# OPM/opm-autodiff

Measured on AMD Instinct MI355X. Metric: Newton iterations/sec, 1M-cell 3-phase black-oil (assembly + ILU0/BiCGStab solve + update), higher is better.
Workload: dtype f64

## Files before the change

### opm-autodiff_amd/csrc/capi.cpp

```cpp
#include <cstdlib>
#include <chrono>
#include <unordered_map>
#include <algorithm>
#include <cstring>
#include <new>

#include "internal.hpp"

using namespace opmhip;

namespace {
thread_local std::string g_err = "";

double now() {
    return std::chrono::duration<double>(std::chrono::steady_clock::now().time_since_epoch()).count();
}

int alloc_system(opmhip_ctx* c) {
    const Pattern& P = c->pat;
    const size_t n = (size_t)P.Nloc * BS;
    int rc;
    constexpr size_t SLACK = 2 * BB;
    if ((rc = dev_alloc(c, &c->d_A, (size_t)P.nnzb * BB + SLACK))) return rc;
    if ((rc = dev_alloc(c, &c->d_L, (size_t)P.nl * BB + SLACK))) return rc;
    if ((rc = dev_alloc(c, &c->d_U, (size_t)P.nu * BB + SLACK))) return rc;
    OPMHIP_HIP(c, hipMemsetAsync(c->d_A + (size_t)P.nnzb * BB, 0, SLACK * sizeof(double), c->stream));
    const size_t l0 = P.fillLevel > 0 ? 0 : (size_t)P.nl * BB, u0 = P.fillLevel > 0 ? 0 : (size_t)P.nu * BB;
    OPMHIP_HIP(c, hipMemsetAsync(c->d_L + l0, 0, ((size_t)P.nl * BB + SLACK - l0) * sizeof(double), c->stream));
    OPMHIP_HIP(c, hipMemsetAsync(c->d_U + u0, 0, ((size_t)P.nu * BB + SLACK - u0) * sizeof(double), c->stream));
    if ((rc = dev_alloc(c, &c->d_invD, (size_t)P.Nb * BB))) return rc;
    c->half_product = half_product_wanted(c);
    if (c->half_product) {
        if ((rc = dev_alloc(c, &c->d_R, (size_t)P.nr * BB + SLACK))) return rc;
        OPMHIP_HIP(c, hipMemsetAsync(c->d_R, 0, ((size_t)P.nr * BB + SLACK) * sizeof(double), c->stream));
        if ((rc = dev_alloc(c, &c->d_usum, n))) return rc;
        OPMHIP_HIP(c, hipMemsetAsync(c->d_usum, 0, n * sizeof(double), c->stream));
    }
    double** vecs[] = {&c->d_b, &c->d_x, &c->d_r, &c->d_rw, &c->d_p, &c->d_v, &c->d_s, &c->d_t, &c->d_pw, &c->d_vu, &c->d_stageV};
    for (double** v : vecs) {
        if ((rc = dev_alloc(c, v, n))) return rc;
        OPMHIP_HIP(c, hipMemsetAsync(*v, 0, n * sizeof(double), c->stream));
    }
    if ((rc = dev_alloc(c, &c->d_stageA, (size_t)P.nnzb * BB))) return rc;
    if ((rc = dev_alloc(c, &c->d_scal, (size_t)SC_COUNT))) return rc;
    OPMHIP_HIP(c, hipMemsetAsync(c->d_scal, 0, SC_COUNT * sizeof(double), c->stream));
    const int vb = (int)((n + 2047) / 2048);
    c->npart = std::max(std::max(P.tiles.ntiles(), P.tiles.nsched), vb) + 1;
    if ((rc = dev_alloc(c, &c->d_part, (size_t)3 * c->npart))) return rc;
    OPMHIP_HIP(c, hipMemsetAsync(c->d_part, 0, (size_t)3 * c->npart * sizeof(double), c->stream));
    if ((rc = dev_alloc(c, &c->d_part2, (size_t)1024))) return rc;
    OPMHIP_HIP(c, hipMemsetAsync(c->d_part2, 0, 1024 * sizeof(double), c->stream));
    if (!c->h_pinned) OPMHIP_HIP(c, hipHostMalloc((void**)&c->h_pinned, SC_COUNT * sizeof(double)));
    if (!c->h_ring) {
    OPMHIP_HIP(c, hipHostMalloc((void**)&c->h_ring, opmhip_ctx::RB_SLOTS * opmhip_ctx::RB_DOUBLES * sizeof(double), hipHostMallocMapped));
    OPMHIP_HIP(c, hipHostGetDevicePointer((void**)&c->d_ring, c->h_ring, 0));
    std::memset(c->h_ring, 0, opmhip_ctx::RB_SLOTS * opmhip_ctx::RB_DOUBLES * sizeof(double));
    }
    c->d_done = c->d_scal + SC_ZERO;
    OPMHIP_HIP(c, hipStreamSynchronize(c->stream));
    return OPMHIP_SUCCESS;
}

static bool no_standard_wells(const opmhip_ctx* c, const opmhip_wells* w) {
    return !w || (w->num_wells <= 0 && !(w->distributed != 0 && c->comm.nranks > 1));
}

static int upload_wells_local(opmhip_ctx* c, const opmhip_wells* w) {
    WellsDev& W = c->wells;
    if (w->num_ms_wells > 0) {
        if (!w->ms_apply) return fail(c, OPMHIP_INVALID_ARGUMENT, "wells: num_ms_wells = %d but ms_apply == NULL", w->num_ms_wells);
        if (c->comm.nranks > 1) return fail(c, OPMHIP_INVALID_ARGUMENT, "wells: multisegment wells through the host callback are not supported in decomposed runs");
        if (W.ms.num > 0)
            return fail(c, OPMHIP_INVALID_ARGUMENT, "wells: num_ms_wells = %d with a callback while a device-resident list of %d multisegment wells is set "
                        "(opmhip_set_ms_wells): the operator would be applied twice", w->num_ms_wells, W.ms.num);
        const size_t bytes = (size_t)c->pat.Nb * BS * sizeof(double);
        if (!W.h_x) OPMHIP_HIP(c, hipHostMalloc((void**)&W.h_x, bytes));
        if (!W.h_y) OPMHIP_HIP(c, hipHostMalloc((void**)&W.h_y, bytes));
        W.num_ms = w->num_ms_wells;
// ... 204 lines not shown
    cfg->tolerance = 1e-2;
    cfg->ilu_relaxation = 0.9;
    cfg->relax_mode = OPMHIP_RELAX_POST_SCALE;
    cfg->reorder = OPMHIP_REORDER_AUTO;
    cfg->cpr_amg_ilu_levels = -1;
    cfg->zero_diag_fix = 1;
    cfg->cpr_reuse_setup = 3;
}

int opmhip_create(const opmhip_config* cfg, opmhip_ctx** out) {
    if (!out) { g_err = "opmhip_create: out == NULL"; return OPMHIP_INVALID_ARGUMENT; }
    *out = nullptr;
    if (!cfg || cfg->abi_version != OPMHIP_ABI_VERSION) { g_err = "opmhip_create: config missing or ABI version mismatch"; return OPMHIP_INVALID_ARGUMENT; }
    if (cfg->maxit < 1 || !(cfg->tolerance > 0.0)) { g_err = "opmhip_create: maxit/tolerance out of range"; return OPMHIP_INVALID_ARGUMENT; }
    if (cfg->preconditioner < OPMHIP_PRECOND_ILU0 || cfg->preconditioner > OPMHIP_PRECOND_CPR_TRUEIMPES) { g_err = "opmhip_create: unknown preconditioner"; return OPMHIP_INVALID_ARGUMENT; }
    if (cfg->chain_length < 0) { g_err = "opmhip_create: chain_length < 0"; return OPMHIP_INVALID_ARGUMENT; }
    if (cfg->cpr_reuse_setup < 0 || cfg->cpr_reuse_setup > 3) { g_err = "opmhip_create: cpr_reuse_setup must be 0 .. 3"; return OPMHIP_INVALID_ARGUMENT; }
    if (cfg->cpr_async_setup < 0 || cfg->cpr_async_setup > 1) { g_err = "opmhip_create: cpr_async_setup must be 0 or 1"; return OPMHIP_INVALID_ARGUMENT; }
    if (cfg->fused_reductions < 0 || cfg->fused_reductions > 1) { g_err = "opmhip_create: fused_reductions must be 0 or 1"; return OPMHIP_INVALID_ARGUMENT; }
    if (cfg->fused_reductions && cfg->tolerance < 1e-6) { g_err = "opmhip_create: fused_reductions needs tolerance >= 1e-6 (the recurred residual norm cannot resolve less than sqrt(eps) |r_0|)"; return OPMHIP_INVALID_ARGUMENT; }
    if (cfg->pin_host_arrays < 0 || cfg->pin_host_arrays > 1) { g_err = "opmhip_create: pin_host_arrays must be 0 or 1"; return OPMHIP_INVALID_ARGUMENT; }
    int ndev = 0;
    hipError_t e = hipGetDeviceCount(&ndev);
    if (e != hipSuccess || ndev <= 0) {
        g_err = std::string("opmhip_create: no HIP device visible (") + hipGetErrorString(e) + "); libopmhip has no CPU fallback";
        return OPMHIP_NO_DEVICE;
    }
    if (cfg->device_id < 0 || cfg->device_id >= ndev) { g_err = "opmhip_create: device_id out of range"; return OPMHIP_INVALID_ARGUMENT; }
    opmhip_ctx* c = new (std::nothrow) opmhip_ctx();
    if (!c) { g_err = "opmhip_create: out of memory"; return OPMHIP_UNKNOWN_ERROR; }
    c->cfg = *cfg;
    c->device = cfg->device_id;
    if ((e = hipSetDevice(c->device)) != hipSuccess || (e = hipStreamCreateWithFlags(&c->stream, hipStreamNonBlocking)) != hipSuccess ||
        (e = hipEventCreate(&c->ev0)) != hipSuccess || (e = hipEventCreate(&c->ev1)) != hipSuccess) {
        g_err = std::string("opmhip_create: ") + hipGetErrorString(e);
        delete c;
        return OPMHIP_DEVICE_ERROR;
    }
    *out = c;
    return OPMHIP_SUCCESS;
}

void opmhip_destroy(opmhip_ctx* c) {
    if (!c) return;
    (void)hipSetDevice(c->device);
    if (c->stream) (void)hipStreamSynchronize(c->stream);
    cpr_shutdown(c);
    comm_release(c);
    for (const auto& r : c->pinned)
        if (r.bytes) (void)hipHostUnregister(const_cast<void*>(r.p));
    for (void* p : c->allocs) (void)hipFree(p);
    if (c->h_pinned) (void)hipHostFree(c->h_pinned);
    if (c->wells.h_x) (void)hipHostFree(c->wells.h_x);
    if (c->wells.h_y) (void)hipHostFree(c->wells.h_y);
    if (c->wells.ms.h_flag) (void)hipHostFree(c->wells.ms.h_flag);
    if (c->h_ring) (void)hipHostFree(c->h_ring);
    if (c->ev0) (void)hipEventDestroy(c->ev0);
    if (c->ev1) (void)hipEventDestroy(c->ev1);
    for (hipEvent_t e : c->prof.ev) (void)hipEventDestroy(e);
    if (c->stream) (void)hipStreamDestroy(c->stream);
    delete c;
}

const char* opmhip_last_error(const opmhip_ctx* c) { return c ? c->err.c_str() : g_err.c_str(); }

int opmhip_synchronize(opmhip_ctx* c) {
    if (!c) return OPMHIP_INVALID_ARGUMENT;
    OPMHIP_HIP(c, hipSetDevice(c->device));
    OPMHIP_HIP(c, hipStreamSynchronize(c->stream));
    return OPMHIP_SUCCESS;
}

int opmhip_set_pattern(opmhip_ctx* c, int Nb, int nnzb, const int* rows, const int* cols) {
    return opmhip_set_pattern_dd(c, Nb, 0, nnzb, rows, cols);
}

int opmhip_set_pattern_dd(opmhip_ctx* c, int Nb, int Nghost, int nnzb, const int* rows, const int* cols) {
    if (!c) return OPMHIP_INVALID_ARGUMENT;
    return guarded(c, [&]() -> int {
        if (c->pattern_set) return fail(c, OPMHIP_NOT_READY, "set_pattern: the pattern of a context is immutable (linalg/ISTLSolverEbos.hpp:216-219)");
        OPMHIP_HIP(c, hipSetDevice(c->device));
        int rc = build_pattern(c, Nb, Nghost, nnzb, rows, cols);
        if (rc) return rc;
        for (int i = 0; i < Nb; ++i)
            if (rows[i + 1] - rows[i] > TILE_CAP_BLOCKS)
                return fail(c, OPMHIP_ANALYSIS_FAILED, "row %d has %d blocks; the ILU0 tile kernel holds at most %d", i, rows[i + 1] - rows[i], TILE_CAP_BLOCKS);
        if ((rc = alloc_system(c))) return rc;
        c->pattern_set = true;
        return OPMHIP_SUCCESS;
    });
}

int opmhip_upload_system(opmhip_ctx* c, const double* vals, const double* b) {
    if (!c) return OPMHIP_INVALID_ARGUMENT;
    return guarded(c, [&]() -> int {
        if (!c->pattern_set) return fail(c, OPMHIP_NOT_READY, "upload_system before set_pattern");
        OPMHIP_HIP(c, hipSetDevice(c->device));
        int rc = upload_system(c, vals, b);
        if (rc) return rc;
        OPMHIP_HIP(c, hipStreamSynchronize(c->stream));
        return OPMHIP_SUCCESS;
    });
// ... 522 lines not shown
    }
    info[3] = P.rest.on ? P.rest.nsched : 0;
    return OPMHIP_SUCCESS;
}

int opmhip_profile_enable(opmhip_ctx* c, int on) {
    if (!c) return OPMHIP_INVALID_ARGUMENT;
    return guarded(c, [&]() -> int {
        OPMHIP_HIP(c, hipSetDevice(c->device));
        OPMHIP_HIP(c, hipStreamSynchronize(c->stream));
        Profiler& P = c->prof;
        P.enabled = on != 0;
        P.every = on > 1 ? on : 1;
        P.solve_no = 0;
        P.suspended = false;
        P.pending = -1;
        P.used = 0;
        P.ev_used = 0;
        for (int k = 0; k < PROF_COUNT; ++k) { P.total_ms[k] = 0.0; P.count[k] = 0; }
        return OPMHIP_SUCCESS;
    });
}

int opmhip_profile_get(opmhip_ctx* c, int cls, long long* launches, double* total_ms) {
    if (!c) return OPMHIP_INVALID_ARGUMENT;
    return guarded(c, [&]() -> int {
        if (cls < 0 || cls >= PROF_COUNT || !launches || !total_ms) return fail(c, OPMHIP_INVALID_ARGUMENT, "profile_get: bad arguments");
        OPMHIP_HIP(c, hipSetDevice(c->device));
        OPMHIP_HIP(c, hipStreamSynchronize(c->stream));
        Profiler& P = c->prof;
        prof_flush(c);
        OPMHIP_HIP(c, hipStreamSynchronize(c->stream));
        if (c->comm.hstream) OPMHIP_HIP(c, hipStreamSynchronize(c->comm.hstream));
        for (size_t i = 0; i < P.used; ++i) {
            float ms = 0.f;
            if (P.cls[i] >= 0 && P.e1[i] >= 0 && hipEventElapsedTime(&ms, P.ev[P.e0[i]], P.ev[P.e1[i]]) == hipSuccess) {
                P.total_ms[P.cls[i]] += ms;
                P.count[P.cls[i]] += 1;
            }
        }
        P.used = 0;
        P.ev_used = 0;
        *launches = P.count[cls];
        *total_ms = P.total_ms[cls];
        return OPMHIP_SUCCESS;
    });
}

int opmhip_cpr_levels(opmhip_ctx* c, int* n, int* nnz, int cap) {
    if (!c || !n || !nnz || cap < 1) return OPMHIP_INVALID_ARGUMENT;
    return cpr_level_sizes(c, n, nnz, cap);
}

int opmhip_time_kernel(opmhip_ctx* c, int which, int reps, double* ms_per_launch) {
    if (!c) return OPMHIP_INVALID_ARGUMENT;
    return guarded(c, [&]() -> int {
        if (!ms_per_launch || reps < 1 || which < 0 || which > 9) return fail(c, OPMHIP_INVALID_ARGUMENT, "time_kernel: bad arguments");
        if (which >= 7 && !c->half_product) return fail(c, OPMHIP_NOT_READY, "time_kernel: the half-product form is not in force on this context");
        if (!c->system_loaded) return fail(c, OPMHIP_NOT_READY, "time_kernel before a matrix was uploaded");
        if (which != 2 && which != 4 && !c->factored) return fail(c, OPMHIP_NOT_READY, "time_kernel: factor first");
        OPMHIP_HIP(c, hipSetDevice(c->device));
        auto once = [&]() {
            switch (which) {
                case 0: (void)launch_spmv(c, c->d_pw, c->d_v, 0, nullptr); break;
                case 1: launch_ilu_apply(c, c->d_p, c->d_pw); break;
                case 2: launch_ilu_factor(c); break;
                case 3: launch_vector_kernels_once(c); break;
                case 4: launch_stream_read(c); break;
                case 5: (void)launch_spmv(c, c->d_pw, c->d_v, 1, c->d_rw); break;
                case 6: (void)launch_spmv(c, c->d_pw, c->d_v, 2, c->d_r); break;
                case 7: (void)launch_spmv(c, c->d_pw, c->d_v, 0, nullptr, 1.0, false, c->d_usum); break;
// ... 20 lines not shown
```

### opm-autodiff_amd/csrc/internal.hpp

```cpp
#pragma once
#include <hip/hip_runtime.h>

#include <cstdarg>
#include <cstdio>
#include <cstdlib>
#include <cstring>
#include <memory>
#include <climits>
#include <string>
#include <type_traits>
#include <vector>

#include "../../include/opmhip.h"
#include "cpr_setup.hpp"

namespace opmhip {

constexpr int BS = 3;
constexpr int BB = 9;

#ifndef OPMHIP_TILE_ROWS
#define OPMHIP_TILE_ROWS 32
#endif
constexpr int TILE_ROWS = OPMHIP_TILE_ROWS;
// ... 239 lines not shown
    double* d_apg = nullptr;
    std::shared_ptr<CprDev> glob;
};
struct CprDev {
    bool structured = false, coarse_direct = true;
    bool level0 = false;
    std::shared_ptr<CprAsyncJob> job;
    bool recreate = false;
    std::vector<CprLevelDev> lv;
    double *d_w = nullptr, *d_lu = nullptr;
    double* d_pcol = nullptr;
    bool w_given = false;
    double *d_r = nullptr, *d_y = nullptr, *d_z = nullptr;
    double omega = 2.0 / 3.0, damp = 1.6, beta = 0.25;
    CprGatherDev gather;
    int apply_rc = 0;
    bool pvals_fresh = false;
};
struct FactorRider {
    int mode = 0;
    double* w = nullptr;
    double* ap = nullptr;
    double* pcol = nullptr;
    int W = 0;
    int ghostFrom = INT_MAX;
};

enum ProfClass { PROF_SPMV = 0, PROF_ILU_APPLY, PROF_ILU_FACTOR, PROF_VECTOR, PROF_ASSEMBLE, PROF_IQ_UPDATE, PROF_CONVERGENCE, PROF_CPR_AMG,
                 PROF_SPMV_BOUNDARY,
                 PROF_HALO,
                 PROF_ALLREDUCE,
                 PROF_CPR_GATHER,
                 PROF_COUNT };
struct Profiler {
    bool enabled = false;
    int every = 1;
    long solve_no = 0;
    bool suspended = false;
    std::vector<hipEvent_t> ev;
    size_t ev_used = 0;
    std::vector<int> cls, e0, e1;
    size_t used = 0;
    int pending = -1;
    bool lazy = false;
    int handoff = -1;
    static constexpr size_t CAP = 1 << 15;
    double total_ms[PROF_COUNT] = {0};
    long count[PROF_COUNT] = {0};
};

enum Scal {
    SC_RHO = 0, SC_RHOP, SC_ALPHA, SC_OMEGA, SC_BETA, SC_TMP1, SC_TMP2, SC_NORM, SC_NORM0,
    SC_DONE,
    SC_ZERO,
    SC_RR,
    SC_RHOH,
    SC_DONEH,
    SC_COUNT = 16
};

}

struct opmhip_ctx {
    opmhip_config cfg;
    int device = 0;
    hipStream_t stream = nullptr;
    hipEvent_t ev0 = nullptr, ev1 = nullptr;
    std::string err;
    bool pattern_set = false, system_loaded = false, factored = false, have_result = false;
    int ilu_fillin = 0;
    opmhip::Pattern pat;
    double *d_A = nullptr, *d_L = nullptr, *d_U = nullptr, *d_invD = nullptr;
    double *d_R = nullptr, *d_usum = nullptr;
    bool half_product = false;
    double *d_b = nullptr, *d_x = nullptr, *d_r = nullptr, *d_rw = nullptr, *d_p = nullptr, *d_v = nullptr,
           *d_s = nullptr, *d_t = nullptr, *d_pw = nullptr, *d_vu = nullptr;
    double *d_stageA = nullptr, *d_stageV = nullptr;
    double* d_scal = nullptr;
    double* d_part = nullptr;
    double minv_scale = 1.0;
    double* d_part2 = nullptr;
    int npart = 0;
    int last_solve_iterations = 0;
    int last_dot_count = 0;
    double* h_pinned = nullptr;
    static constexpr int RB_SLOTS = 4, RB_DOUBLES = 4;
    double* h_ring = nullptr;
    double* d_ring = nullptr;
    double rb_seq = 0.0;
    double rb_want[RB_SLOTS] = {0, 0, 0, 0};
    const double* d_done = nullptr;
    opmhip::WellsDev wells;
    opmhip::AsmDev asmb;
    opmhip::CommDev comm;
    opmhip::CprDev cpr;
    opmhip::Profiler prof;
    std::vector<void*> allocs;
    struct HostRange { const void* p; size_t bytes; };
    std::vector<HostRange> pinned;
};

namespace opmhip {

inline const char* tuning_env(const char* name) {
    static const bool on = [] { const char* e = std::getenv("OPMHIP_TUNING"); return e && e[0] == '1'; }();
    const char* v = std::getenv(name);
    if (!v) return nullptr;
    if (!on) {
        std::fprintf(stderr, "opmhip: %s is set but OPMHIP_TUNING=1 is not - ignored\n", name);
        return nullptr;
    }
    std::fprintf(stderr, "opmhip: measurement switch %s=%s is in force\n", name, v);
    return v;
// ... 20 lines not shown
inline bool poison_allocations() {
    static const bool on = [] { const char* e = tuning_env("OPMHIP_POISON_ALLOC"); return e && e[0] == '1'; }();
    return on;
}
template <class T>
int dev_alloc(opmhip_ctx* c, T** p, size_t count) {
    void* q = nullptr;
    size_t bytes = (count ? count : 1) * sizeof(T);
    hipError_t e = hipMalloc(&q, bytes);
    if (e != hipSuccess)
        return fail(c, OPMHIP_DEVICE_ERROR, "hipMalloc(%zu) failed: %s", bytes, hipGetErrorString(e));
    if (poison_allocations() && ((e = hipMemset(q, std::is_floating_point<T>::value ? 0xFF : 0x00, bytes)) != hipSuccess || (e = hipDeviceSynchronize()) != hipSuccess)) {
        (void)hipFree(q);
        return fail(c, OPMHIP_DEVICE_ERROR, "hipMemset(%zu) failed: %s", bytes, hipGetErrorString(e));
    }
    c->allocs.push_back(q);
    *p = static_cast<T*>(q);
    return OPMHIP_SUCCESS;
}
template <class T>
void dev_free(opmhip_ctx* c, T** p) {
    if (!*p) return;
    for (size_t i = 0; i < c->allocs.size(); ++i)
        if (c->allocs[i] == (void*)*p) { c->allocs[i] = c->allocs.back(); c->allocs.pop_back(); break; }
    (void)hipFree((void*)*p);
    *p = nullptr;
}
template <class T>
int dev_upload(opmhip_ctx* c, T** p, const std::vector<T>& h) {
    int rc = dev_alloc(c, p, h.size());
    if (rc) return rc;
    if (!h.empty()) OPMHIP_HIP(c, hipMemcpy(*p, h.data(), h.size() * sizeof(T), hipMemcpyHostToDevice));
    return OPMHIP_SUCCESS;
}

inline int prof_event(opmhip_ctx* c, hipStream_t s = nullptr) {
    Profiler& P = c->prof;
    if (P.ev.size() <= P.ev_used) {
        hipEvent_t e;
        if (hipEventCreate(&e) != hipSuccess) return -1;
        P.ev.push_back(e);
    }
    const int i = (int)P.ev_used++;
    (void)hipEventRecord(P.ev[i], s ? s : c->stream);
    return i;
}
inline int prof_event_slot(opmhip_ctx* c) {
    Profiler& P = c->prof;
    if (P.ev.size() <= P.ev_used) {
        hipEvent_t e;
        if (hipEventCreate(&e) != hipSuccess) return -1;
        P.ev.push_back(e);
    }
    return (int)P.ev_used++;
}
inline void prof_flush(opmhip_ctx* c) {
    Profiler& P = c->prof;
    P.handoff = -1;
    if (P.pending < 0) return;
    const int e = prof_event(c);
    if (e >= 0) P.e1[P.pending] = e; else P.cls[P.pending] = -1;
    P.pending = -1;
}
inline int prof_begin(opmhip_ctx* c, int cls) {
    Profiler& P = c->prof;
    if (!P.enabled || P.suspended || P.used >= Profiler::CAP) { prof_flush(c); return -1; }
// ... 109 lines not shown
```

### opm-autodiff_amd/csrc/solver.hip

```cpp
#include <hip/hip_runtime.h>
#include <hip/hip_ext.h>
#include <atomic>

#include <chrono>
#include <cmath>
#include <cstdlib>

#include "internal.hpp"

namespace opmhip {

#ifndef OPMHIP_STAGE_DEPTH
#define OPMHIP_STAGE_DEPTH 16
#endif
typedef double v2d_t __attribute__((ext_vector_type(2)));
__device__ __forceinline__ double2 ld_stream(const double2* p) {
    const v2d_t t = __builtin_nontemporal_load(reinterpret_cast<const v2d_t*>(p));
    return make_double2(t.x, t.y);
}
__device__ __forceinline__ void st_rowsum(double* p, double v) {
    __builtin_nontemporal_store(v, p);
}
__device__ __forceinline__ void stage_doubles(const double* __restrict__ src, double* __restrict__ dst, int n, int lane) {
    const double2* __restrict__ s2 = reinterpret_cast<const double2*>(src);
// ... 1639 lines not shown
#pragma unroll
    for (int u = 0; u < VPT; ++u) {
        const int e = base + u * VB;
        if (e < n) p[e] = (p[e] - omega * __builtin_nontemporal_load(&v[e])) * beta + r[e];
    }
}
template <bool SR = false>
__global__ __launch_bounds__(VB) void k_bicg_upd1(int n, const double* __restrict__ scal, double* __restrict__ r,
                                                  const double* __restrict__ v, double* __restrict__ part, int npart, double half = -1.0) {
    if (scal[SC_DONE] != 0.0 && !(SR && scal[SC_DONEH] == half)) return;
    const double alpha = scal[SC_ALPHA];
    double s = 0.0;
    const int base = blockIdx.x * VB * VPT + threadIdx.x;
#pragma unroll
    for (int u = 0; u < VPT; ++u) {
        const int e = base + u * VB;
        if (e < n) {
            const double re = r[e] - alpha * __builtin_nontemporal_load(&v[e]);
            r[e] = re;
            s += re * re;
        }
    }
    if (!SR) block_partials(s, 0.0, part, npart, 1);
}
__global__ __launch_bounds__(VB) void k_bicg_xhalf(int n, const double* __restrict__ scal, double* __restrict__ x, const double* __restrict__ pw, double ws) {
    const double alpha = scal[SC_ALPHA];
    const int base = blockIdx.x * VB * VPT + threadIdx.x;
#pragma unroll
    for (int u = 0; u < VPT; ++u) {
        const int e = base + u * VB;
        if (e < n) x[e] += alpha * (ws * pw[e]);
    }
}
template <bool SR = false>
__global__ __launch_bounds__(VB) void k_bicg_upd2(int n, const double* __restrict__ scal, double* __restrict__ x,
                                                  const double* __restrict__ pw, const double* __restrict__ sv, double* __restrict__ r,
                                                  const double* __restrict__ tv, const double* __restrict__ rw,
                                                  double* __restrict__ part, int npart, double ws, double half = -1.0) {
    if (scal[SC_DONE] != 0.0 && !(SR && scal[SC_DONEH] == half)) return;
    const double alpha = scal[SC_ALPHA], omega = scal[SC_OMEGA];
    double s = 0.0, q = 0.0;
    const int base = blockIdx.x * VB * VPT + threadIdx.x;
#pragma unroll
    for (int u = 0; u < VPT; ++u) {
        const int e = base + u * VB;
        if (e < n) {
            const double xh = __builtin_nontemporal_load(&x[e]) + alpha * (ws * __builtin_nontemporal_load(&pw[e]));
            __builtin_nontemporal_store(xh + omega * (ws * __builtin_nontemporal_load(&sv[e])), &x[e]);
            const double re = r[e] - omega * __builtin_nontemporal_load(&tv[e]);
            r[e] = re;
            s += re * re;
            q += rw[e] * re;
        }
    }
    if (!SR) block_partials(s, q, part, npart, 2);
}
__global__ __launch_bounds__(VB) void k_dots(int n, const double* __restrict__ a, const double* __restrict__ b,
                                             double* __restrict__ part, int npart, int nsum) {
    double s = 0.0, q = 0.0;
    const int base = blockIdx.x * VB * VPT + threadIdx.x;
#pragma unroll
    for (int u = 0; u < VPT; ++u) {
        const int e = base + u * VB;
        if (e < n) { s += a[e] * b[e]; q += a[e] * a[e]; }
    }
    block_partials(s, q, part, npart, nsum);
// ... 599 lines not shown
        prof_span_end(c, span);
        if (rc) return rc;
        hipLaunchKernelGGL(k_finalize, dim3(1), dim3(VB), 0, c->stream, mode, 1, c->comm.d_red, 1, c->d_scal, tol, hslot, seq);
        return OPMHIP_SUCCESS;
    }
    if (count > RED1_SINGLE_MAX) {
        hipLaunchKernelGGL(k_reduce_finalize, dim3(RED1_BLOCKS), dim3(VB), 0, c->stream, mode, count, c->d_part, c->npart, c->d_part2,
                           reinterpret_cast<unsigned*>(c->d_part2 + 2 * RED1_BLOCKS), c->d_scal, tol, hslot, seq);
        return OPMHIP_SUCCESS;
    }
    hipLaunchKernelGGL(k_finalize, dim3(1), dim3(VB), 0, c->stream, mode, count, c->d_part, c->npart, c->d_scal, tol, hslot, seq);
    return OPMHIP_SUCCESS;
}
static int finalize3(opmhip_ctx* c, int mode, int count, int rb_half) {
    const double tol = c->cfg.tolerance;
    const int sl = rb_half % opmhip_ctx::RB_SLOTS;
    double* hslot = c->d_ring + (size_t)sl * opmhip_ctx::RB_DOUBLES;
    const double seq = (c->rb_seq += 1.0);
    c->rb_want[sl] = seq;
    if (c->comm.nranks > 1) {
        const int span = prof_span_begin(c, PROF_ALLREDUCE);
        hipLaunchKernelGGL(k_finalize3, dim3(1), dim3(VB), 0, c->stream, (int)FIN_LOCAL, count, c->d_part, c->npart, c->comm.d_red, tol, (double*)nullptr, 0.0, 0.0);
        c->comm.reduce_span_open = true;
        const int rc = comm_allreduce(c, c->comm.d_red, 3, 0);
        c->comm.reduce_span_open = false;
        prof_span_end(c, span);
        if (rc) return rc;
        hipLaunchKernelGGL(k_finalize3, dim3(1), dim3(VB), 0, c->stream, mode, 1, c->comm.d_red, 1, c->d_scal, tol, hslot, seq, (double)rb_half);
        return OPMHIP_SUCCESS;
    }
    hipLaunchKernelGGL(k_finalize3, dim3(1), dim3(VB), 0, c->stream, mode, count, c->d_part, c->npart, c->d_scal, tol, hslot, seq, (double)rb_half);
    return OPMHIP_SUCCESS;
}
void launch_vector_kernels_once(opmhip_ctx* c) {
    const int n = c->pat.Nb * BS, nb = vec_blocks(n);
    hipLaunchKernelGGL(k_bicg_pupdate, dim3(nb), dim3(VB), 0, c->stream, n, c->d_scal, c->d_p, c->d_v, c->d_r);
    hipLaunchKernelGGL(k_bicg_upd1<false>, dim3(nb), dim3(VB), 0, c->stream, n, c->d_scal, c->d_r, c->d_v, c->d_part, c->npart, -1.0);
    (void)finalize(c, FIN_NORM, nb);
    hipLaunchKernelGGL(k_bicg_upd2<false>, dim3(nb), dim3(VB), 0, c->stream, n, c->d_scal, c->d_x, c->d_pw, c->d_s, c->d_r, c->d_t, c->d_rw, c->d_part, c->npart, c->minv_scale, -1.0);
    (void)finalize(c, FIN_NORM_RHO, nb);
}

static int read_scalars(opmhip_ctx* c) {
    OPMHIP_HIP(c, hipMemcpyAsync(c->h_pinned, c->d_scal, SC_COUNT * sizeof(double), hipMemcpyDeviceToHost, c->stream));
    OPMHIP_HIP(c, hipStreamSynchronize(c->stream));
    return OPMHIP_SUCCESS;
}
enum { HALF_ALL = 0, HALF_PRECOND = 1, HALF_REST = 2 };
static int enqueue_half(opmhip_ctx* c, int h, int part = HALF_ALL) {
    const Pattern& P = c->pat;
    const int n = P.Nb * BS, nb = vec_blocks(n);
    const bool cpr = use_cpr(c);
    const bool hp = !cpr && c->half_product;
    const bool sr = c->cfg.fused_reductions > 0;
    const bool precTalks = cpr && c->cpr.gather.on;
    const bool head = part != HALF_REST, rest = part != HALF_PRECOND;
    const bool applyNow = part == HALF_ALL || (precTalks ? part == HALF_REST : part == HALF_PRECOND);
    int rc, ps;
    if ((h & 1) == 0) {
        if (head && h > 0) {
            ps = prof_begin(c, PROF_VECTOR);
            hipLaunchKernelGGL(k_bicg_pupdate, dim3(nb), dim3(VB), 0, c->stream, n, c->d_scal, c->d_p, c->d_v, c->d_r);
            prof_end(c, ps);
        }
        if (applyNow) {
            if (cpr) launch_cpr_apply(c, c->d_p, c->d_pw);
            else launch_ilu_apply(c, c->d_p, c->d_pw, -1.0, &c->minv_scale, nullptr, nullptr, hp ? c->d_usum : nullptr);
            if (cpr && c->cpr.apply_rc) { rc = c->cpr.apply_rc; c->cpr.apply_rc = 0; return rc; }
        }
        if (!rest) return OPMHIP_SUCCESS;
        if (sr) {
            if ((rc = launch_spmv(c, c->d_pw, c->d_v, 3, c->d_rw, c->minv_scale, true, hp ? c->d_usum : nullptr, c->d_r))) return rc;
            ps = prof_begin(c, PROF_VECTOR);
            if ((rc = finalize3(c, FIN_SR1, dot_count(c), h))) return rc;
            hipLaunchKernelGGL(k_bicg_upd1<true>, dim3(nb), dim3(VB), 0, c->stream, n, c->d_scal, c->d_r, c->d_v, c->d_part, c->npart, (double)h);
            prof_end(c, ps);
            return OPMHIP_SUCCESS;
        }
        if ((rc = launch_spmv(c, c->d_pw, c->d_v, 1, c->d_rw, c->minv_scale, true, hp ? c->d_usum : nullptr))) return rc;
        ps = prof_begin(c, PROF_VECTOR);
        if ((rc = finalize(c, FIN_ALPHA, dot_count(c)))) return rc;
        hipLaunchKernelGGL(k_bicg_upd1<false>, dim3(nb), dim3(VB), 0, c->stream, n, c->d_scal, c->d_r, c->d_v, c->d_part, c->npart, -1.0);
        if ((rc = finalize(c, FIN_NORM, nb, h))) return rc;
        prof_end(c, ps);
    } else {
        if (applyNow) {
            if (cpr) launch_cpr_apply(c, c->d_r, c->d_s);
            else launch_ilu_apply(c, c->d_r, c->d_s, -1.0, &c->minv_scale, nullptr, nullptr, hp ? c->d_usum : nullptr);
            if (cpr && c->cpr.apply_rc) { rc = c->cpr.apply_rc; c->cpr.apply_rc = 0; return rc; }
        }
        if (!rest) return OPMHIP_SUCCESS;
        if (sr) {
            if ((rc = launch_spmv(c, c->d_s, c->d_t, 3, c->d_r, c->minv_scale, true, hp ? c->d_usum : nullptr, c->d_rw))) return rc;
            ps = prof_begin(c, PROF_VECTOR);
            if ((rc = finalize3(c, FIN_SR2, dot_count(c), h))) return rc;
            hipLaunchKernelGGL(k_bicg_upd2<true>, dim3(nb), dim3(VB), 0, c->stream, n, c->d_scal, c->d_x, c->d_pw, c->d_s, c->d_r, c->d_t, c->d_rw, c->d_part, c->npart, c->minv_scale, (double)h);
            prof_end(c, ps);
            return OPMHIP_SUCCESS;
        }
        if ((rc = launch_spmv(c, c->d_s, c->d_t, 2, c->d_r, c->minv_scale, true, hp ? c->d_usum : nullptr))) return rc;
        ps = prof_begin(c, PROF_VECTOR);
        if ((rc = finalize(c, FIN_OMEGA, dot_count(c)))) return rc;
        hipLaunchKernelGGL(k_bicg_upd2<false>, dim3(nb), dim3(VB), 0, c->stream, n, c->d_scal, c->d_x, c->d_pw, c->d_s, c->d_r, c->d_t, c->d_rw, c->d_part, c->npart, c->minv_scale, -1.0);
        if ((rc = finalize(c, FIN_NORM_RHO, nb, h))) return rc;
        prof_end(c, ps);
    }
    return OPMHIP_SUCCESS;
}
static int wait_half(opmhip_ctx* c, int h, double* norm, double* norm_0) {
    const int sl = h % opmhip_ctx::RB_SLOTS;
    const volatile double* slot = c->h_ring + (size_t)sl * opmhip_ctx::RB_DOUBLES;
    const double want = c->rb_want[sl];
    const auto t0 = std::chrono::steady_clock::now();
    for (unsigned long spin = 1;; ++spin) {
        if (slot[3] == want) break;
        if ((spin & 0xFFFFu) == 0) {
            const hipError_t e = hipStreamQuery(c->stream);
            if (e == hipSuccess) {
                if (slot[3] == want) break;
                return fail(c, OPMHIP_DEVICE_ERROR, "BiCGStab: the stream drained without the stopping-rule record of half iteration %d", h);
            }
            if (e != hipErrorNotReady) return fail(c, OPMHIP_DEVICE_ERROR, "BiCGStab: %s", hipGetErrorString(e));
            if (std::chrono::steady_clock::now() - t0 > std::chrono::seconds(120))
                return fail(c, OPMHIP_DEVICE_ERROR, "BiCGStab: no stopping-rule record of half iteration %d after 120 s", h);
        }
#if defined(__x86_64__) || defined(__i386__)
        __builtin_ia32_pause();
#elif defined(__aarch64__)
        asm volatile("yield" ::: "memory");
#endif
    }
    std::atomic_thread_fence(std::memory_order_acquire);
    *norm = slot[0];
    *norm_0 = slot[1];
    return OPMHIP_SUCCESS;
}
int bicgstab(opmhip_ctx* c, opmhip_result* res) {
    const Pattern& P = c->pat;
    const int n = P.Nb * BS, nb = vec_blocks(n);
    const int maxit = c->cfg.maxit;
    const double tol = c->cfg.tolerance;
    struct SolveScope {
        opmhip_ctx* c;
        explicit SolveScope(opmhip_ctx* c_) : c(c_) {
            c->d_done = c->d_scal + SC_DONE;
            Profiler& Q = c->prof;
            Q.solve_no += 1;
            Q.suspended = Q.enabled && Q.every > 1 && (Q.solve_no % Q.every) != 0;
            Q.lazy = c->comm.nranks == 1;
        }
        ~SolveScope() {
            c->d_done = c->d_scal + SC_ZERO;
            c->prof.lazy = false;
            prof_flush(c);
            c->prof.suspended = false;
        }
    } scope(c);
    int rc;
    c->minv_scale = 1.0;
    hipLaunchKernelGGL(k_bicg_init, dim3(nb), dim3(VB), 0, c->stream, n, c->d_b, c->d_r, c->d_rw, c->d_p, c->d_x, c->d_v, c->d_part, c->npart);
    if ((rc = finalize(c, FIN_INIT, nb))) return rc;
    const int nhalves = 2 * maxit;
    double norm = 0.0, norm_0 = 0.0;
    float it = maxit + 0.5f;
    size_t mark_next = c->prof.used;
    const bool split = c->comm.nranks > 1;
    if (nhalves > 0 && (rc = enqueue_half(c, 0))) return rc;
    for (int h = 0; h < nhalves; ++h) {
        mark_next = c->prof.used;
        if (h + 1 < nhalves && (rc = enqueue_half(c, h + 1, split ? HALF_PRECOND : HALF_ALL))) return rc;
        if ((rc = wait_half(c, h, &norm, &norm_0))) return rc;
        if (!std::isfinite(norm)) {
            prof_flush(c);
            break;
        }
        if (norm < tol * norm_0) {
            it = 0.5f * (float)(h + 1);
            prof_flush(c);
            for (size_t i = mark_next; i < c->prof.used; ++i) c->prof.cls[i] = -1;
            if ((h & 1) == 0) hipLaunchKernelGGL(k_bicg_xhalf, dim3(nb), dim3(VB), 0, c->stream, n, c->d_scal, c->d_x, c->d_pw, c->minv_scale);
            break;
        }
        if (split && h + 1 < nhalves && (rc = enqueue_half(c, h + 1, HALF_REST))) return rc;
    }
    if (nhalves <= 0) {
        if ((rc = read_scalars(c))) return rc;
        norm = norm_0 = c->h_pinned[SC_NORM0];
    }
    bool drifted = false;
    if (c->cfg.fused_reductions > 0 && nhalves > 0 && std::isfinite(norm)) {
        hipLaunchKernelGGL(k_dots, dim3(nb), dim3(VB), 0, c->stream, n, c->d_r, c->d_r, c->d_part, c->npart, 1);
        if ((rc = finalize(c, FIN_TRUE, nb))) return rc;
        if ((rc = read_scalars(c))) return rc;
        const double truth = c->h_pinned[SC_TMP1];
        drifted = it != (maxit + 0.5f) && !(truth < 2.0 * tol * norm_0);
        norm = truth;
    }
    OPMHIP_HIP(c, hipGetLastError());
    res->it = it;
    res->iterations = (int)std::fmin(it, (float)maxit);
    res->reduction = norm / norm_0;
    res->conv_rate = std::pow(res->reduction, 1.0 / it);
    res->converged = (it != (maxit + 0.5f)) && !drifted;
    return OPMHIP_SUCCESS;
}

}
```

Baseline: 86.06.

## Overlap BiCGStab solution update on a side stream with double-buffered pw/s

Splits the second BiCGStab update kernel into a residual update with dot partials on the main stream and a solution (x) update on a separate stream. The x update reads alpha/omega from a per-parity record and uses double-buffered pw/s vectors, so the next preconditioner apply can proceed while x is still being updated. Events join the side stream before buffers are reused and at solve end. This aims to take the x read-modify-write off the critical path, but it adds event overhead, extra memory for two vectors, and contention when both streams run bandwidth-bound kernels at once.

After: 83.27. 0.968x the previous value.

```diff
diff --git a/opm-autodiff_amd/csrc/capi.cpp b/opm-autodiff_amd/csrc/capi.cpp
--- a/opm-autodiff_amd/csrc/capi.cpp
+++ b/opm-autodiff_amd/csrc/capi.cpp
@@ -36,7 +36,7 @@
         if ((rc = dev_alloc(c, &c->d_usum, n))) return rc;
         OPMHIP_HIP(c, hipMemsetAsync(c->d_usum, 0, n * sizeof(double), c->stream));
     }
-    double** vecs[] = {&c->d_b, &c->d_x, &c->d_r, &c->d_rw, &c->d_p, &c->d_v, &c->d_s, &c->d_t, &c->d_pw, &c->d_vu, &c->d_stageV};
+    double** vecs[] = {&c->d_b, &c->d_x, &c->d_r, &c->d_rw, &c->d_p, &c->d_v, &c->d_s, &c->d_t, &c->d_pw, &c->d_vu, &c->d_stageV, &c->d_pw1, &c->d_s1};
     for (double** v : vecs) {
         if ((rc = dev_alloc(c, v, n))) return rc;
         OPMHIP_HIP(c, hipMemsetAsync(*v, 0, n * sizeof(double), c->stream));
@@ -44,6 +44,8 @@
     if ((rc = dev_alloc(c, &c->d_stageA, (size_t)P.nnzb * BB))) return rc;
     if ((rc = dev_alloc(c, &c->d_scal, (size_t)SC_COUNT))) return rc;
     OPMHIP_HIP(c, hipMemsetAsync(c->d_scal, 0, SC_COUNT * sizeof(double), c->stream));
+    if ((rc = dev_alloc(c, &c->d_xrec, (size_t)2 * opmhip_ctx::XREC_DOUBLES))) return rc;
+    OPMHIP_HIP(c, hipMemsetAsync(c->d_xrec, 0, 2 * opmhip_ctx::XREC_DOUBLES * sizeof(double), c->stream));
     const int vb = (int)((n + 2047) / 2048);
     c->npart = std::max(std::max(P.tiles.ntiles(), P.tiles.nsched), vb) + 1;
     if ((rc = dev_alloc(c, &c->d_part, (size_t)3 * c->npart))) return rc;
@@ -314,9 +316,12 @@
     c->cfg = *cfg;
     c->device = cfg->device_id;
     if ((e = hipSetDevice(c->device)) != hipSuccess || (e = hipStreamCreateWithFlags(&c->stream, hipStreamNonBlocking)) != hipSuccess ||
-        (e = hipEventCreate(&c->ev0)) != hipSuccess || (e = hipEventCreate(&c->ev1)) != hipSuccess) {
+        (e = hipEventCreate(&c->ev0)) != hipSuccess || (e = hipEventCreate(&c->ev1)) != hipSuccess ||
+        (e = hipStreamCreateWithFlags(&c->xstream, hipStreamNonBlocking)) != hipSuccess ||
+        (e = hipEventCreateWithFlags(&c->ev_r[0], hipEventDisableTiming)) != hipSuccess || (e = hipEventCreateWithFlags(&c->ev_r[1], hipEventDisableTiming)) != hipSuccess ||
+        (e = hipEventCreateWithFlags(&c->ev_x[0], hipEventDisableTiming)) != hipSuccess || (e = hipEventCreateWithFlags(&c->ev_x[1], hipEventDisableTiming)) != hipSuccess) {
         g_err = std::string("opmhip_create: ") + hipGetErrorString(e);
-        delete c;
+        opmhip_destroy(c);
         return OPMHIP_DEVICE_ERROR;
     }
     *out = c;
@@ -327,6 +332,7 @@
     if (!c) return;
     (void)hipSetDevice(c->device);
     if (c->stream) (void)hipStreamSynchronize(c->stream);
+    if (c->xstream) (void)hipStreamSynchronize(c->xstream);
     cpr_shutdown(c);
     comm_release(c);
     for (const auto& r : c->pinned)
@@ -340,6 +346,9 @@
     if (c->ev0) (void)hipEventDestroy(c->ev0);
     if (c->ev1) (void)hipEventDestroy(c->ev1);
     for (hipEvent_t e : c->prof.ev) (void)hipEventDestroy(e);
+    for (hipEvent_t e : {c->ev_r[0], c->ev_r[1], c->ev_x[0], c->ev_x[1]})
+        if (e) (void)hipEventDestroy(e);
+    if (c->xstream) (void)hipStreamDestroy(c->xstream);
     if (c->stream) (void)hipStreamDestroy(c->stream);
     delete c;
 }
@@ -350,6 +359,7 @@
     if (!c) return OPMHIP_INVALID_ARGUMENT;
     OPMHIP_HIP(c, hipSetDevice(c->device));
     OPMHIP_HIP(c, hipStreamSynchronize(c->stream));
+    OPMHIP_HIP(c, hipStreamSynchronize(c->xstream));
     return OPMHIP_SUCCESS;
 }
 
@@ -938,11 +948,13 @@
         prof_flush(c);
         OPMHIP_HIP(c, hipStreamSynchronize(c->stream));
         if (c->comm.hstream) OPMHIP_HIP(c, hipStreamSynchronize(c->comm.hstream));
+        OPMHIP_HIP(c, hipStreamSynchronize(c->xstream));
         for (size_t i = 0; i < P.used; ++i) {
             float ms = 0.f;
             if (P.cls[i] >= 0 && P.e1[i] >= 0 && hipEventElapsedTime(&ms, P.ev[P.e0[i]], P.ev[P.e1[i]]) == hipSuccess) {
-                P.total_ms[P.cls[i]] += ms;
-                P.count[P.cls[i]] += 1;
+                const int k = P.cls[i] & ~PROF_TIME_ONLY;
+                P.total_ms[k] += ms;
+                if (!(P.cls[i] & PROF_TIME_ONLY)) P.count[k] += 1;
             }
         }
         P.used = 0;
diff --git a/opm-autodiff_amd/csrc/internal.hpp b/opm-autodiff_amd/csrc/internal.hpp
--- a/opm-autodiff_amd/csrc/internal.hpp
+++ b/opm-autodiff_amd/csrc/internal.hpp
@@ -295,6 +295,7 @@
                  PROF_ALLREDUCE,
                  PROF_CPR_GATHER,
                  PROF_COUNT };
+constexpr int PROF_TIME_ONLY = 1 << 8;
 struct Profiler {
     bool enabled = false;
     int every = 1;
@@ -342,6 +343,13 @@
     double* d_scal = nullptr;
     double* d_part = nullptr;
     double minv_scale = 1.0;
+    double *d_pw1 = nullptr, *d_s1 = nullptr;
+    double* d_xrec = nullptr;
+    static constexpr int XREC_DOUBLES = 4;
+    hipStream_t xstream = nullptr;
+    hipEvent_t ev_r[2] = {nullptr, nullptr};
+    hipEvent_t ev_x[2] = {nullptr, nullptr};
+    bool x_inflight[2] = {false, false};
     double* d_part2 = nullptr;
     int npart = 0;
     int last_solve_iterations = 0;
@@ -428,6 +436,13 @@
     if (rc) return rc;
     if (!h.empty()) OPMHIP_HIP(c, hipMemcpy(*p, h.data(), h.size() * sizeof(T), hipMemcpyHostToDevice));
     return OPMHIP_SUCCESS;
+}
+
+inline double* solve_pw(const opmhip_ctx* c, int h) { return ((h >> 1) & 1) ? c->d_pw1 : c->d_pw; }
+inline double* solve_s(const opmhip_ctx* c, int h) { return ((h >> 1) & 1) ? c->d_s1 : c->d_s; }
+inline void join_xstream(opmhip_ctx* c) {
+    for (int k = 0; k < 2; ++k)
+        if (c->x_inflight[k]) { (void)hipStreamWaitEvent(c->stream, c->ev_x[k], 0); c->x_inflight[k] = false; }
 }
 
 inline int prof_event(opmhip_ctx* c, hipStream_t s = nullptr) {
diff --git a/opm-autodiff_amd/csrc/solver.hip b/opm-autodiff_amd/csrc/solver.hip
--- a/opm-autodiff_amd/csrc/solver.hip
+++ b/opm-autodiff_amd/csrc/solver.hip
@@ -1695,6 +1695,40 @@
         if (e < n) x[e] += alpha * (ws * pw[e]);
     }
 }
+__global__ __launch_bounds__(VB) void k_bicg_rupd2(int n, const double* __restrict__ scal, double* __restrict__ r, const double* __restrict__ tv,
+                                                   const double* __restrict__ rw, double* __restrict__ part, int npart, double* __restrict__ rec) {
+    const bool go = scal[SC_DONE] == 0.0;
+    const double omega = scal[SC_OMEGA];
+    if (blockIdx.x == 0 && threadIdx.x == 0) { rec[0] = scal[SC_ALPHA]; rec[1] = omega; rec[2] = go ? 1.0 : 0.0; }
+    if (!go) return;
+    double s = 0.0, q = 0.0;
+    const int base = blockIdx.x * VB * VPT + threadIdx.x;
+#pragma unroll
+    for (int u = 0; u < VPT; ++u) {
+        const int e = base + u * VB;
+        if (e < n) {
+            const double re = r[e] - omega * __builtin_nontemporal_load(&tv[e]);
+            r[e] = re;
+            s += re * re;
+            q += rw[e] * re;
+        }
+    }
+    block_partials(s, q, part, npart, 2);
+}
+__global__ __launch_bounds__(VB) void k_bicg_xupd(int n, const double* __restrict__ rec, double* __restrict__ x, const double* __restrict__ pw,
+                                                  const double* __restrict__ sv, double ws) {
+    if (rec[2] == 0.0) return;
+    const double alpha = rec[0], omega = rec[1];
+    const int base = blockIdx.x * VB * VPT + threadIdx.x;
+#pragma unroll
+    for (int u = 0; u < VPT; ++u) {
+        const int e = base + u * VB;
+        if (e < n) {
+            const double xh = __builtin_nontemporal_load(&x[e]) + alpha * (ws * __builtin_nontemporal_load(&pw[e]));
+            __builtin_nontemporal_store(xh + omega * (ws * __builtin_nontemporal_load(&sv[e])), &x[e]);
+        }
+    }
+}
 template <bool SR = false>
 __global__ __launch_bounds__(VB) void k_bicg_upd2(int n, const double* __restrict__ scal, double* __restrict__ x,
                                                   const double* __restrict__ pw, const double* __restrict__ sv, double* __restrict__ r,
@@ -2360,12 +2394,25 @@
     hipLaunchKernelGGL(k_finalize3, dim3(1), dim3(VB), 0, c->stream, mode, count, c->d_part, c->npart, c->d_scal, tol, hslot, seq, (double)rb_half);
     return OPMHIP_SUCCESS;
 }
+static void launch_second_updates(opmhip_ctx* c, int h) {
+    const int n = c->pat.Nb * BS, nb = vec_blocks(n), k = (h >> 1) & 1;
+    double* rec = c->d_xrec + (size_t)k * opmhip_ctx::XREC_DOUBLES;
+    hipLaunchKernelGGL(k_bicg_rupd2, dim3(nb), dim3(VB), 0, c->stream, n, c->d_scal, c->d_r, c->d_t, c->d_rw, c->d_part, c->npart, rec);
+    (void)hipEventRecord(c->ev_r[k], c->stream);
+    (void)hipStreamWaitEvent(c->xstream, c->ev_r[k], 0);
+    const int span = prof_span_begin(c, PROF_VECTOR | PROF_TIME_ONLY, c->xstream);
+    hipLaunchKernelGGL(k_bicg_xupd, dim3(nb), dim3(VB), 0, c->xstream, n, rec, c->d_x, solve_pw(c, h), solve_s(c, h), c->minv_scale);
+    prof_span_end(c, span, c->xstream);
+    (void)hipEventRecord(c->ev_x[k], c->xstream);
+    c->x_inflight[k] = true;
+}
 void launch_vector_kernels_once(opmhip_ctx* c) {
     const int n = c->pat.Nb * BS, nb = vec_blocks(n);
     hipLaunchKernelGGL(k_bicg_pupdate, dim3(nb), dim3(VB), 0, c->stream, n, c->d_scal, c->d_p, c->d_v, c->d_r);
     hipLaunchKernelGGL(k_bicg_upd1<false>, dim3(nb), dim3(VB), 0, c->stream, n, c->d_scal, c->d_r, c->d_v, c->d_part, c->npart, -1.0);
     (void)finalize(c, FIN_NORM, nb);
-    hipLaunchKernelGGL(k_bicg_upd2<false>, dim3(nb), dim3(VB), 0, c->stream, n, c->d_scal, c->d_x, c->d_pw, c->d_s, c->d_r, c->d_t, c->d_rw, c->d_part, c->npart, c->minv_scale, -1.0);
+    hipLaunchKernelGGL(k_bicg_rupd2, dim3(nb), dim3(VB), 0, c->stream, n, c->d_scal, c->d_r, c->d_t, c->d_rw, c->d_part, c->npart, c->d_xrec);
+    hipLaunchKernelGGL(k_bicg_xupd, dim3(nb), dim3(VB), 0, c->stream, n, c->d_xrec, c->d_x, c->d_pw, c->d_s, c->minv_scale);
     (void)finalize(c, FIN_NORM_RHO, nb);
 }
 
@@ -2384,6 +2431,7 @@
     const bool precTalks = cpr && c->cpr.gather.on;
     const bool head = part != HALF_REST, rest = part != HALF_PRECOND;
     const bool applyNow = part == HALF_ALL || (precTalks ? part == HALF_REST : part == HALF_PRECOND);
+    double *pw = solve_pw(c, h), *sv = solve_s(c, h);
     int rc, ps;
     if ((h & 1) == 0) {
         if (head && h > 0) {
@@ -2392,20 +2440,22 @@
             prof_end(c, ps);
         }
         if (applyNow) {
-            if (cpr) launch_cpr_apply(c, c->d_p, c->d_pw);
-            else launch_ilu_apply(c, c->d_p, c->d_pw, -1.0, &c->minv_scale, nullptr, nullptr, hp ? c->d_usum : nullptr);
+            const int k = (h >> 1) & 1;
+            if (c->x_inflight[k]) { (void)hipStreamWaitEvent(c->stream, c->ev_x[k], 0); c->x_inflight[k] = false; }
+            if (cpr) launch_cpr_apply(c, c->d_p, pw);
+            else launch_ilu_apply(c, c->d_p, pw, -1.0, &c->minv_scale, nullptr, nullptr, hp ? c->d_usum : nullptr);
             if (cpr && c->cpr.apply_rc) { rc = c->cpr.apply_rc; c->cpr.apply_rc = 0; return rc; }
         }
         if (!rest) return OPMHIP_SUCCESS;
         if (sr) {
-            if ((rc = launch_spmv(c, c->d_pw, c->d_v, 3, c->d_rw, c->minv_scale, true, hp ? c->d_usum : nullptr, c->d_r))) return rc;
+            if ((rc = launch_spmv(c, pw, c->d_v, 3, c->d_rw, c->minv_scale, true, hp ? c->d_usum : nullptr, c->d_r))) return rc;
             ps = prof_begin(c, PROF_VECTOR);
             if ((rc = finalize3(c, FIN_SR1, dot_count(c), h))) return rc;
             hipLaunchKernelGGL(k_bicg_upd1<true>, dim3(nb), dim3(VB), 0, c->stream, n, c->d_scal, c->d_r, c->d_v, c->d_part, c->npart, (double)h);
             prof_end(c, ps);
             return OPMHIP_SUCCESS;
         }
-        if ((rc = launch_spmv(c, c->d_pw, c->d_v, 1, c->d_rw, c->minv_scale, true, hp ? c->d_usum : nullptr))) return rc;
+        if ((rc = launch_spmv(c, pw, c->d_v, 1, c->d_rw, c->minv_scale, true, hp ? c->d_usum : nullptr))) return rc;
         ps = prof_begin(c, PROF_VECTOR);
         if ((rc = finalize(c, FIN_ALPHA, dot_count(c)))) return rc;
         hipLaunchKernelGGL(k_bicg_upd1<false>, dim3(nb), dim3(VB), 0, c->stream, n, c->d_scal, c->d_r, c->d_v, c->d_part, c->npart, -1.0);
@@ -2413,23 +2463,23 @@
         prof_end(c, ps);
     } else {
         if (applyNow) {
-            if (cpr) launch_cpr_apply(c, c->d_r, c->d_s);
-            else launch_ilu_apply(c, c->d_r, c->d_s, -1.0, &c->minv_scale, nullptr, nullptr, hp ? c->d_usum : nullptr);
+            if (cpr) launch_cpr_apply(c, c->d_r, sv);
+            else launch_ilu_apply(c, c->d_r, sv, -1.0, &c->minv_scale, nullptr, nullptr, hp ? c->d_usum : nullptr);
             if (cpr && c->cpr.apply_rc) { rc = c->cpr.apply_rc; c->cpr.apply_rc = 0; return rc; }
         }
         if (!rest) return OPMHIP_SUCCESS;
         if (sr) {
-            if ((rc = launch_spmv(c, c->d_s, c->d_t, 3, c->d_r, c->minv_scale, true, hp ? c->d_usum : nullptr, c->d_rw))) return rc;
+            if ((rc = launch_spmv(c, sv, c->d_t, 3, c->d_r, c->minv_scale, true, hp ? c->d_usum : nullptr, c->d_rw))) return rc;
             ps = prof_begin(c, PROF_VECTOR);
             if ((rc = finalize3(c, FIN_SR2, dot_count(c), h))) return rc;
-            hipLaunchKernelGGL(k_bicg_upd2<true>, dim3(nb), dim3(VB), 0, c->stream, n, c->d_scal, c->d_x, c->d_pw, c->d_s, c->d_r, c->d_t, c->d_rw, c->d_part, c->npart, c->minv_scale, (double)h);
+            hipLaunchKernelGGL(k_bicg_upd2<true>, dim3(nb), dim3(VB), 0, c->stream, n, c->d_scal, c->d_x, pw, sv, c->d_r, c->d_t, c->d_rw, c->d_part, c->npart, c->minv_scale, (double)h);
             prof_end(c, ps);
             return OPMHIP_SUCCESS;
         }
-        if ((rc = launch_spmv(c, c->d_s, c->d_t, 2, c->d_r, c->minv_scale, true, hp ? c->d_usum : nullptr))) return rc;
+        if ((rc = launch_spmv(c, sv, c->d_t, 2, c->d_r, c->minv_scale, true, hp ? c->d_usum : nullptr))) return rc;
         ps = prof_begin(c, PROF_VECTOR);
         if ((rc = finalize(c, FIN_OMEGA, dot_count(c)))) return rc;
-        hipLaunchKernelGGL(k_bicg_upd2<false>, dim3(nb), dim3(VB), 0, c->stream, n, c->d_scal, c->d_x, c->d_pw, c->d_s, c->d_r, c->d_t, c->d_rw, c->d_part, c->npart, c->minv_scale, -1.0);
+        launch_second_updates(c, h);
         if ((rc = finalize(c, FIN_NORM_RHO, nb, h))) return rc;
         prof_end(c, ps);
     }
@@ -2478,6 +2528,7 @@
             Q.lazy = c->comm.nranks == 1;
         }
         ~SolveScope() {
+            join_xstream(c);
             c->d_done = c->d_scal + SC_ZERO;
             c->prof.lazy = false;
             prof_flush(c);
@@ -2506,7 +2557,10 @@
             it = 0.5f * (float)(h + 1);
             prof_flush(c);
             for (size_t i = mark_next; i < c->prof.used; ++i) c->prof.cls[i] = -1;
-            if ((h & 1) == 0) hipLaunchKernelGGL(k_bicg_xhalf, dim3(nb), dim3(VB), 0, c->stream, n, c->d_scal, c->d_x, c->d_pw, c->minv_scale);
+            if ((h & 1) == 0) {
+                join_xstream(c);
+                hipLaunchKernelGGL(k_bicg_xhalf, dim3(nb), dim3(VB), 0, c->stream, n, c->d_scal, c->d_x, solve_pw(c, h), c->minv_scale);
+            }
             break;
         }
         if (split && h + 1 < nhalves && (rc = enqueue_half(c, h + 1, HALF_REST))) return rc;
@@ -2515,6 +2569,7 @@
         if ((rc = read_scalars(c))) return rc;
         norm = norm_0 = c->h_pinned[SC_NORM0];
     }
+    join_xstream(c);
     bool drifted = false;
     if (c->cfg.fused_reductions > 0 && nhalves > 0 && std::isfinite(norm)) {
         hipLaunchKernelGGL(k_dots, dim3(nb), dim3(VB), 0, c->stream, n, c->d_r, c->d_r, c->d_part, c->npart, 1);
```
